# p-m-mueller/saddle_point_petsc

Hardware: AMD Instinct MI355X
Metric: FGMRES iterations/sec + achieved HBM GB/s on A-block SpMV, 1/2/4/8 MI355X (higher is better)
Workload: dtype f64

## Files before the change

### saddle_point_petsc_amd/csrc/spk_dict.hpp

```cpp
#pragma once
#include "spk_device.hpp"

namespace spk {
namespace k {

constexpr int kDictChunk = kThreads;
constexpr int kDictG3 = 9;
constexpr int kDict2Wgs = 512;
typedef int int2v __attribute__((ext_vector_type(2)));
typedef unsigned long long u64;

struct DictArgs {
    const uint16_t *tid;
    const int32_t *tab;
    const double *cls;
    const int32_t *fld;
    const unsigned char *codes;
    const double *zpad;
    int32_t nbrows, ntype, nclass, kmax;
    int32_t nchunks, chunks_per_xcd, chunks_per_wg;
    int32_t tab_ints, cls_off, fld_off;
    int64_t plane_off[kDictMaxK];
    int32_t strad;
    int32_t u3l[9], u3r[9];
    int32_t uw[4];
};

__device__ __forceinline__ void dict_load_lds(const DictArgs &d, int nclsvals, char *smem)
{
    int32_t *ti = reinterpret_cast<int32_t *>(smem);
    for (int i = threadIdx.x; i < d.tab_ints; i += blockDim.x) ti[i] = d.tab[i];
    double2 *cv = reinterpret_cast<double2 *>(smem + d.cls_off);
    const double2 *src = reinterpret_cast<const double2 *>(d.cls);
    for (int i = threadIdx.x; i < nclsvals; i += blockDim.x) cv[i] = src[i];
    int32_t *fl = reinterpret_cast<int32_t *>(smem + d.fld_off);
    for (int i = threadIdx.x; i < nclsvals; i += blockDim.x) fl[i] = d.fld[i];
    __syncthreads();
}
struct DictTables {
    const int32_t *tlen;
    int2 *tent;
    const double2 *cv;
    const int32_t *fl;
};
__device__ __forceinline__ DictTables dict_tables(const DictArgs &d, char *smem)
{
    return DictTables{reinterpret_cast<const int32_t *>(smem), reinterpret_cast<int2 *>(smem + 4 * ((d.ntype + 1) & ~1)),
                      reinterpret_cast<const double2 *>(smem + d.cls_off), reinterpret_cast<const int32_t *>(smem + d.fld_off)};
}
__device__ __forceinline__ bool dict_chunk_range(const DictArgs &d, int bx, int &c0, int &c1)
{
    c0 = ((bx & 7) * d.chunks_per_xcd + (bx >> 3) * d.chunks_per_wg);
    c1 = min(min(c0 + d.chunks_per_wg, ((bx & 7) + 1) * d.chunks_per_xcd), d.nchunks);
    return c0 < c1;
}
template <int KM>
__device__ __forceinline__ void dict_prepare_types(const DictArgs &d, const DictTables &T, int stride)
{
    for (int i = threadIdx.x; i < d.ntype * KM; i += kThreads) {
        const int t = i / KM, k = i - t * KM;
        int2 e = T.tent[i];
        if (k < T.tlen[t]) e.x *= stride;
        else e = make_int2((int)0x80000000u, d.nclass);
        T.tent[i] = e;
    }
    __syncthreads();
}
__device__ __forceinline__ int dict_rowof(const DictArgs &d, int ch) { return min(ch * kDictChunk + (int)threadIdx.x, d.nbrows - 1); }

__device__ __forceinline__ void dict_issue_pair2(const DictArgs &d, int p, int64_t br, u64 &w0, u64 &w1)
{
    const unsigned char *base = d.codes + d.plane_off[p];
    if (2 * p + 1 < d.kmax) {
        const int4v r = __builtin_nontemporal_load(reinterpret_cast<const int4v *>(base) + br);
        w0 = (u64)(uint32_t)r.x | ((u64)(uint32_t)r.y << 32);
        w1 = (u64)(uint32_t)r.z | ((u64)(uint32_t)r.w << 32);
    } else {
        const int2v r = __builtin_nontemporal_load(reinterpret_cast<const int2v *>(base) + br);
        w0 = (u64)(uint32_t)r.x | ((u64)(uint32_t)r.y << 32);
        w1 = 0ull;
    }
}
__device__ __forceinline__ void dict_issue3(const DictArgs &d, int k, int64_t br, u64 &w0, u64 &w1)
{
    const int4v r = __builtin_nontemporal_load(reinterpret_cast<const int4v *>(d.codes + d.plane_off[k]) + br);
    w0 = (u64)(uint32_t)r.x | ((u64)(uint32_t)r.y << 32);
    w1 = (u64)(uint32_t)r.z | ((u64)(uint32_t)r.w << 32);
}
__device__ __forceinline__ int dict_field(u64 w0, u64 w1, int fd)
{
    const u64 w = (fd >> 16) ? w1 : w0;
    const int sh = fd & 255, wd = (fd >> 8) & 255;
    return (int)((long long)(w << (64 - sh - wd)) >> (64 - wd));
}
template <int SPLIT>
__device__ __forceinline__ constexpr bool dict3_in_w1(int e)
{
    return SPLIT == 1 ? e >= 5 : SPLIT == 2 ? e >= 4 : (e == 4 || e >= 6);
}
template <int SPLIT>
__device__ __forceinline__ int dict_field3u(u64 w0, u64 w1, const DictArgs &d, int e)
{
    const u64 w = dict3_in_w1<SPLIT>(e) ? w1 : w0;
    return (int)((long long)(w << d.u3l[e]) >> 32) >> d.u3r[e];
}
__device__ __forceinline__ int dict_field2(u64 w, int fd)
{
    const int lo = (int)(uint32_t)w, hi = (int)(uint32_t)(w >> 32);
    const int mask = fd >> 31;
    const int src = (hi & mask) | (lo & ~mask);
    return __builtin_amdgcn_sbfe(src, (unsigned)fd, (unsigned)(fd >> 8));
}
constexpr int kDictAcross = 1 << 30;
__device__ __forceinline__ int dict_field2(u64 w, int fd, bool strad)
{
    if (strad && (fd & kDictAcross)) {
        const int sh = fd & 63, wd = (fd >> 8) & 31;
        return (int)((long long)(w << (64 - sh - wd)) >> (64 - wd));
    }
    return dict_field2(w, fd);
}
__device__ __forceinline__ double dict_decode(int code, double2 bs)
{
    return __builtin_fma((double)code, bs.y, bs.x);
}
template <int BS>
__device__ __forceinline__ u64 *dict_word_ptr(const DictArgs &d, unsigned char *codes, int k, int64_t br)
{
    if (BS == 3) return reinterpret_cast<u64 *>(codes + d.plane_off[k]) + 2 * br;
    const int p = k >> 1;
    if (2 * p + 1 < d.kmax) return reinterpret_cast<u64 *>(codes + d.plane_off[p]) + 2 * br + (k & 1);
    return reinterpret_cast<u64 *>(codes + d.plane_off[p]) + br;
}

inline DictArgs dict_args(const DictDev &A, int *grid)
{
    DictArgs d{};
    d.tid = A.tid.p;
    d.tab = A.tab.p;
    d.cls = A.cls.p;
    d.fld = A.fld.p;
    d.codes = A.codes.p;
    d.zpad = A.zpad.p;
    d.strad = A.straddle ? 1 : 0;
    for (int e = 0; e < 9; ++e) {
        d.u3l[e] = A.u3l[e];
        d.u3r[e] = A.u3r[e];
    }
    for (int e = 0; e < 4; ++e) d.uw[e] = A.uniform ? A.uw[e] : 0;
    d.nbrows = A.nbrows;
    d.ntype = A.ntype;
    d.nclass = A.nclass;
    d.kmax = A.kmax;
    d.nchunks = (A.nbrows + kDictChunk - 1) / kDictChunk;
    static const int wgs2 = [] { const char *e = getenv("SPK_DICT2_WGS"); return e && atoi(e) > 0 ? atoi(e) : kDict2Wgs; }();
    d.chunks_per_wg = std::max(1, d.nchunks / (A.bs == 2 && A.kmax == 9 ? wgs2 : 2048));
    const int cpx = (d.nchunks + 7) / 8;
    d.chunks_per_xcd = (cpx + d.chunks_per_wg - 1) / d.chunks_per_wg * d.chunks_per_wg;
    d.tab_ints = ((A.ntype + 1) & ~1) + 2 * A.ntype * A.kmax;
    d.cls_off = (4 * d.tab_ints + 15) & ~15;
    d.fld_off = d.cls_off + 16 * (A.nclass + 1) * A.bs * A.bs;
    for (int k = 0; k < kDictMaxK; ++k) d.plane_off[k] = A.plane_off[k];
    *grid = 8 * (d.chunks_per_xcd / d.chunks_per_wg);
    return d;
}

}
}
```

### saddle_point_petsc_amd/csrc/spk_k_dict.hip

```cpp
#include "spk_dict.hpp"

#include <climits>

namespace spk {
namespace k {

template <int BS, bool ACC, bool RIDE, bool BT, int U3>
__global__ __launch_bounds__(kThreads) void spmv_dict_kernel(DictArgs d, const double *__restrict__ x, double *__restrict__ y,
                                                             RowTail tail, const int32_t *__restrict__ done, GivensRider gr)
{
#pragma clang fp contract(off)
    extern __shared__ __attribute__((aligned(16))) char smem[];
    const int bx = product_prologue<RIDE>(done, gr, reinterpret_cast<double *>(smem));
    int c0, c1;
    if (bx < 0 || !dict_chunk_range(d, bx, c0, c1)) return;
    int br = c0 * kDictChunk + (int)threadIdx.x;
    int tidn = br < d.nbrows ? (int)d.tid[br] : -1;
    dict_load_lds(d, (d.nclass + 1) * BS * BS, smem);
    const DictTables T = dict_tables(d, smem);

    for (int ch = c0; ch < c1; ++ch) {
        const int tc = tidn;
        const int brc = br;
        br += kDictChunk;
        tidn = (ch + 1 < c1 && br < d.nbrows) ? (int)d.tid[br] : -1;
        if (tc < 0) continue;
        double s[BS];
#pragma unroll
        for (int r = 0; r < BS; ++r) s[r] = 0.0;
        double yacc[BS];
        if (ACC) {
            if (BS == 2) {
                const double2 t = reinterpret_cast<const double2 *>(y)[brc];
                yacc[0] = t.x;
                yacc[1] = t.y;
            } else {
#pragma unroll
                for (int r = 0; r < BS; ++r) yacc[r] = y[(int64_t)BS * brc + r];
            }
        }
        BtPre pre[BS];
        if (BT) {
#pragma unroll
            for (int r = 0; r < BS; ++r) pre[r].load(tail, (int64_t)BS * brc + r);
        }
        const int len = T.tlen[tc];
        const int2 *te = T.tent + (size_t)tc * d.kmax;
        constexpr int G = BS == 2 ? 10 : kDictG3;
        for (int k0 = 0; k0 < len; k0 += G) {
            int2 e[G];
            u64 w0[G], w1[BS == 2 ? 1 : G];
            double xv[G][BS];
            if (BS == 2) {
#pragma unroll
                for (int h = 0; h < G / 2; ++h) {
                    w0[2 * h] = w0[2 * h + 1] = 0ull;
                    if (k0 + 2 * h < len) dict_issue_pair2(d, (k0 >> 1) + h, brc, w0[2 * h], w0[2 * h + 1]);
                }
            }
#pragma unroll
            for (int g = 0; g < G; ++g) {
                const bool in = k0 + g < len;
                e[g] = in ? te[k0 + g] : make_int2(0, 0);
                if (in) {
                    if (BS == 3) dict_issue3(d, k0 + g, brc, w0[g], w1[BS == 2 ? 0 : g]);
                    const int64_t c = (int64_t)brc + e[g].x;
                    if (BS == 2) {
                        const double2 t = reinterpret_cast<const double2 *>(x)[c];
                        xv[g][0] = t.x;
                        xv[g][1] = t.y;
                    } else {
#pragma unroll
                        for (int j = 0; j < BS; ++j) xv[g][j] = x[BS * c + j];
                    }
                }
            }
#pragma unroll
            for (int g = 0; g < G; ++g) {
                if (k0 + g < len) {
                    const double2 *cb = T.cv + (size_t)e[g].y * (BS * BS);
                    const int32_t *fb = T.fl + (size_t)e[g].y * (BS * BS);
#pragma unroll
                    for (int r = 0; r < BS; ++r)
#pragma unroll
                        for (int j = 0; j < BS; ++j)
                            s[r] += dict_decode(BS == 2 ? dict_field2(w0[g], fb[r * BS + j], d.strad != 0)
                                                       : U3 ? dict_field3u<(U3 ? U3 : 1)>(w0[g], w1[BS == 2 ? 0 : g], d, r * BS + j)
                                                            : dict_field(w0[g], w1[BS == 2 ? 0 : g], fb[r * BS + j]),
                                                cb[r * BS + j]) * xv[g][j];
                }
            }
        }
#pragma unroll
        for (int r = 0; r < BS; ++r) {
            row_tail_add(tail, (int64_t)BS * brc + r, s[r], false);
            if (BT) pre[r].add(tail, s[r]);
            if (ACC) s[r] += yacc[r];
        }
        if (BS == 2) {
            double2 o;
            o.x = s[0];
            o.y = s[1];
            reinterpret_cast<double2 *>(y)[brc] = o;
        } else {
#pragma unroll
            for (int r = 0; r < BS; ++r) y[(int64_t)BS * brc + r] = s[r];
        }
    }
}

template <int KM, bool ACC>
struct Dict2Stage {
    u64 w[KM + 1];
    double2 xv[KM];
    int cls[KM];
    double2 yv;
};

template <int KM, bool ACC>
__device__ __forceinline__ void dict2_issue(const DictArgs &d, __amdgpu_buffer_rsrc_t xr, const double *__restrict__ y,
                                            const int2 *tent, int tc, int brr, Dict2Stage<KM, ACC> &S)
{
    static_assert(KM % 2 == 1, "an odd last position: its plane holds single words");
#pragma unroll
    for (int h = 0; h < KM / 2; ++h) {
        const int4v r = __builtin_nontemporal_load(reinterpret_cast<const int4v *>(d.codes + d.plane_off[h]) + brr);
        S.w[2 * h] = (u64)(uint32_t)r.x | ((u64)(uint32_t)r.y << 32);
        S.w[2 * h + 1] = (u64)(uint32_t)r.z | ((u64)(uint32_t)r.w << 32);
    }
    {
        const int2v r = __builtin_nontemporal_load(reinterpret_cast<const int2v *>(d.codes + d.plane_off[KM / 2]) + brr);
        S.w[KM - 1] = (u64)(uint32_t)r.x | ((u64)(uint32_t)r.y << 32);
    }
    if (ACC) S.yv = reinterpret_cast<const double2 *>(y)[brr];
    const int2 *te = tent + (size_t)tc * KM;
    const uint32_t b16 = (uint32_t)brr * 16u;
#pragma unroll
    for (int g = 0; g < KM; ++g) {
        const int2 e = te[g];
        S.cls[g] = e.y;
        const int4v r = __builtin_bit_cast(int4v, __builtin_amdgcn_raw_buffer_load_b128(xr, (int)(b16 + (uint32_t)e.x), 0, 0));
        S.xv[g].x = __hiloint2double(r.y, r.x);
        S.xv[g].y = __hiloint2double(r.w, r.z);
    }
}

template <bool ACC, bool RIDE, bool BT, int KM, bool UNI>
__global__ __launch_bounds__(kThreads) void spmv_dict2_kernel(DictArgs d, const double *__restrict__ x, double *__restrict__ y,
                                                              RowTail tail, const int32_t *__restrict__ done, GivensRider gr)
{
#pragma clang fp contract(off)
    extern __shared__ __attribute__((aligned(16))) char smem[];
    const int bx = product_prologue<RIDE>(done, gr, reinterpret_cast<double *>(smem));
    int c0, c1;
    if (bx < 0 || !dict_chunk_range(d, bx, c0, c1)) return;
    int tA = (int)d.tid[dict_rowof(d, c0)];
    int tB = (int)d.tid[dict_rowof(d, c0 + 1)];
    dict_load_lds(d, (d.nclass + 1) * 4, smem);
    const DictTables T = dict_tables(d, smem);
    dict_prepare_types<KM>(d, T, 16);
    const __amdgpu_buffer_rsrc_t xr = __builtin_amdgcn_make_buffer_rsrc(const_cast<double *>(x), 0, 16 * d.nbrows, 0x00020000);

    Dict2Stage<KM, ACC> SA, SB;
    auto compute = [&](int ch, const Dict2Stage<KM, ACC> &S) {
        const int brc = ch * kDictChunk + (int)threadIdx.x;
        double s[2] = {0.0, 0.0};
#pragma unroll
        for (int g = 0; g < KM; ++g) {
            const double2 *cb = T.cv + (size_t)S.cls[g] * 4;
            if (UNI) {
                const int lo = (int)(uint32_t)S.w[g], hi = (int)(uint32_t)(S.w[g] >> 32);
                s[0] += dict_decode(__builtin_amdgcn_sbfe(lo, 0u, (unsigned)d.uw[0]), cb[0]) * S.xv[g].x;
                s[0] += dict_decode(lo >> (32 - d.uw[1]), cb[1]) * S.xv[g].y;
                s[1] += dict_decode(__builtin_amdgcn_sbfe(hi, 0u, (unsigned)d.uw[2]), cb[2]) * S.xv[g].x;
                s[1] += dict_decode(hi >> (32 - d.uw[3]), cb[3]) * S.xv[g].y;
            } else {
                const int32_t *fb = T.fl + (size_t)S.cls[g] * 4;
                s[0] += dict_decode(dict_field2(S.w[g], fb[0]), cb[0]) * S.xv[g].x;
                s[0] += dict_decode(dict_field2(S.w[g], fb[1]), cb[1]) * S.xv[g].y;
                s[1] += dict_decode(dict_field2(S.w[g], fb[2]), cb[2]) * S.xv[g].x;
                s[1] += dict_decode(dict_field2(S.w[g], fb[3]), cb[3]) * S.xv[g].y;
            }
        }
        if (brc >= d.nbrows) return;
#pragma unroll
        for (int r = 0; r < 2; ++r) {
            row_tail_add(tail, 2 * (int64_t)brc + r, s[r], BT);
            if (ACC) s[r] += r == 0 ? S.yv.x : S.yv.y;
        }
        double2 o;
        o.x = s[0];
        o.y = s[1];
        reinterpret_cast<double2 *>(y)[brc] = o;
    };

    dict2_issue<KM, ACC>(d, xr, y, T.tent, tA, dict_rowof(d, c0), SA);
    tA = (int)d.tid[dict_rowof(d, c0 + 2)];
    for (int ch = c0;; ch += 2) {
        dict2_issue<KM, ACC>(d, xr, y, T.tent, tB, dict_rowof(d, ch + 1), SB);
        tB = (int)d.tid[dict_rowof(d, ch + 3)];
        compute(ch, SA);
        if (ch + 1 >= c1) break;
        dict2_issue<KM, ACC>(d, xr, y, T.tent, tA, dict_rowof(d, ch + 2), SA);
        tA = (int)d.tid[dict_rowof(d, ch + 4)];
        compute(ch + 1, SB);
        if (ch + 2 >= c1) break;
    }
}

void spmv_dict(const DictDev &A, const double *x, double *y, const CsrDev *bt, const double *lam, const int32_t *done,
               hipStream_t s, bool accumulate, const OffDiag *odp, const GivensRider *rider)
{
    if (product_is_empty(A.nbrows, rider, done, s)) return;
    if (spmv_dict3(A, x, y, bt, lam, done, s, accumulate, odp, rider)) return;
    const ProductLaunch p = make_product_launch(bt, lam, odp, rider, done, accumulate);
    int grid = 0;
    const DictArgs d = dict_args(A, &grid);
    const size_t lds = std::max((size_t)A.lds_bytes, p.rider_lds);
    const bool pipelined = A.bs == 2 && A.kmax == 9 && A.nbrows < (1 << 27) && !A.straddle;
    dispatch_product(p.acc, p.ride, p.bt, [&](auto acc, auto ride, auto btf) {
        constexpr bool ACC = acc.value, RIDE = ride.value, BTF = btf.value;
        auto launch = [&](auto kern) {
            SPK_LAUNCH_PRODUCT(kern, dim3(grid + p.nride), dim3(kThreads), lds, s, d, x, y, p.tail, p.done, p.gr);
        };
        if (pipelined && A.uniform) launch(spmv_dict2_kernel<ACC, RIDE, BTF, 9, true>);
        else if (pipelined) launch(spmv_dict2_kernel<ACC, RIDE, BTF, 9, false>);
        else if (A.bs == 2) launch(spmv_dict_kernel<2, ACC, RIDE, BTF, 0>);
        else if (A.uniform3 == 0) launch(spmv_dict_kernel<3, ACC, RIDE, BTF, 0>);
        else if (A.uniform3 == 1) launch(spmv_dict_kernel<3, ACC, RIDE, BTF, 1>);
        else if (A.uniform3 == 2) launch(spmv_dict_kernel<3, ACC, RIDE, BTF, 2>);
        else launch(spmv_dict_kernel<3, ACC, RIDE, BTF, 3>);
    });
}

template <int BS, int U3>
__global__ __launch_bounds__(kThreads) void jacobi_sweep_f32_dict_kernel(DictArgs d, const float *__restrict__ d32, float omega,
                                                                         const float *__restrict__ x32,
                                                                         const float *__restrict__ yin, float *__restrict__ yout,
                                                                         const int32_t *__restrict__ done)
{
#pragma clang fp contract(off)
    if (done && *done) return;
    extern __shared__ __attribute__((aligned(16))) char smem[];
    int c0, c1;
    if (!dict_chunk_range(d, (int)blockIdx.x, c0, c1)) return;
    dict_load_lds(d, (d.nclass + 1) * BS * BS, smem);
    const DictTables T = dict_tables(d, smem);
    for (int ch = c0; ch < c1; ++ch) {
        const int br = ch * kDictChunk + (int)threadIdx.x;
        if (br >= d.nbrows) continue;
        const int tc = (int)d.tid[br];
        float s[BS];
#pragma unroll
        for (int r = 0; r < BS; ++r) s[r] = 0.0f;
        const int len = T.tlen[tc];
        const int2 *te = T.tent + (size_t)tc * d.kmax;
        constexpr int G = BS == 2 ? 10 : 3;
        for (int k0 = 0; k0 < len; k0 += G) {
            int2 e[G];
            u64 w0[G], w1[BS == 2 ? 1 : G];
            float yv[G][BS];
            if (BS == 2) {
#pragma unroll
                for (int h = 0; h < G / 2; ++h) {
                    w0[2 * h] = w0[2 * h + 1] = 0ull;
                    if (k0 + 2 * h < len) dict_issue_pair2(d, (k0 >> 1) + h, br, w0[2 * h], w0[2 * h + 1]);
                }
            }
#pragma unroll
            for (int g = 0; g < G; ++g) {
                const bool in = k0 + g < len;
                e[g] = in ? te[k0 + g] : make_int2(0, 0);
                if (in) {
                    if (BS == 3) dict_issue3(d, k0 + g, br, w0[g], w1[BS == 2 ? 0 : g]);
                    const int64_t c = (int64_t)br + e[g].x;
#pragma unroll
                    for (int j = 0; j < BS; ++j) yv[g][j] = yin[BS * c + j];
                }
            }
#pragma unroll
            for (int g = 0; g < G; ++g) {
                if (k0 + g < len) {
                    const double2 *cb = T.cv + (size_t)e[g].y * (BS * BS);
                    const int32_t *fb = T.fl + (size_t)e[g].y * (BS * BS);
#pragma unroll
                    for (int r = 0; r < BS; ++r)
#pragma unroll
                        for (int j = 0; j < BS; ++j)
                            s[r] = (s[r] + ((float)dict_decode(BS == 2 ? dict_field2(w0[g], fb[r * BS + j], d.strad != 0)
                                                                      : U3 ? dict_field3u<(U3 ? U3 : 1)>(w0[g], w1[BS == 2 ? 0 : g], d, r * BS + j)
                                                                           : dict_field(w0[g], w1[BS == 2 ? 0 : g], fb[r * BS + j]),
                                                               cb[r * BS + j]) * yv[g][j]));
                }
            }
        }
#pragma unroll
        for (int r = 0; r < BS; ++r) {
            const int64_t row = (int64_t)BS * br + r;
            yout[row] = sweep_update(yin[row], omega, d32[row], x32[row], s[r]);
        }
    }
}

void jacobi_sweep_f32_dict(const DictDev &A, const float *d32, float omega, const float *x32, const float *yin, float *yout,
                           const int32_t *done, hipStream_t s)
{
    if (A.nbrows == 0) return;
    if (jacobi_sweep_f32_dict3(A, d32, omega, x32, yin, yout, done, s)) return;
    int grid = 0;
    const DictArgs d = dict_args(A, &grid);
#define SPK_LAUNCH_SWEEP(BS, U3)                                                                                                \
    hipLaunchKernelGGL((jacobi_sweep_f32_dict_kernel<BS, U3>), dim3(grid), dim3(kThreads), (size_t)A.lds_bytes, s, d, d32, omega, x32, \
                       yin, yout, done)
    if (A.bs == 2) SPK_LAUNCH_SWEEP(2, 0);
    else if (A.uniform3 == 0) SPK_LAUNCH_SWEEP(3, 0);
    else if (A.uniform3 == 1) SPK_LAUNCH_SWEEP(3, 1);
    else if (A.uniform3 == 2) SPK_LAUNCH_SWEEP(3, 2);
    else SPK_LAUNCH_SWEEP(3, 3);
#undef SPK_LAUNCH_SWEEP
}

__device__ __forceinline__ unsigned long long mix64(unsigned long long h, unsigned long long w)
{
    h ^= w + 0x9E3779B97F4A7C15ull + (h << 6) + (h >> 2);
    h *= 0xBF58476D1CE4E5B9ull;
    h ^= h >> 31;
    return h;
}
__device__ __forceinline__ int dict_insert(unsigned long long h, int32_t item, unsigned long long *keys, int32_t *rep,
                                           int32_t *ctl, int maxkeys)
{
    if (h == 0ull) h = 1ull;
    int idx = (int)(h & (unsigned long long)(kDictSlots - 1));
    for (int probe = 0; probe < kDictSlots; ++probe) {
        if (__hip_atomic_load(ctl + 1, __ATOMIC_RELAXED, __HIP_MEMORY_SCOPE_AGENT)) return -1;
        unsigned long long prev = __hip_atomic_load(keys + idx, __ATOMIC_RELAXED, __HIP_MEMORY_SCOPE_AGENT);
        if (prev == 0ull) {
            prev = atomicCAS(keys + idx, 0ull, h);
            if (prev == 0ull && atomicAdd(ctl, 1) + 1 > maxkeys) {
                __hip_atomic_store(ctl + 1, 1, __ATOMIC_RELAXED, __HIP_MEMORY_SCOPE_AGENT);
                return -1;
            }
        }
        if (prev == 0ull || prev == h) {
            if (item < __hip_atomic_load(rep + idx, __ATOMIC_RELAXED, __HIP_MEMORY_SCOPE_AGENT)) atomicMin(rep + idx, item);
            return idx;
        }
        idx = (idx + 1) & (kDictSlots - 1);
    }
    __hip_atomic_store(ctl + 1, 1, __ATOMIC_RELAXED, __HIP_MEMORY_SCOPE_AGENT);
    return -1;
}

template <int BS>
__device__ __forceinline__ double blk_val(const double *v0, const double *v1, int64_t ldp, int64_t q, int r, int j)
{
    if (BS == 2) return (r == 0 ? v0 : v1)[2 * q + j];
    return v0[(int64_t)(3 * r + j) * ldp + q];
}
__device__ __forceinline__ unsigned long long coarse_key(double v)
{
    if (!(fabs(v) < 1e12)) return (unsigned long long)__double_as_longlong(v);
    return (unsigned long long)(long long)rint(v * 1048576.0);
}

template <int BS>
__global__ __launch_bounds__(kThreads) void dict_hash_blocks_kernel(const double *__restrict__ v0, const double *__restrict__ v1,
                                                                    int64_t ldp, int64_t nblocks, unsigned long long *keys,
                                                                    int32_t *rep, int32_t *slot, int32_t *ctl, int maxkeys)
{
    const int64_t q = (int64_t)blockIdx.x * kThreads + threadIdx.x;
    if (q >= nblocks) return;
    unsigned long long h = 0x243F6A8885A308D3ull;
#pragma unroll
    for (int r = 0; r < BS; ++r)
#pragma unroll
        for (int j = 0; j < BS; ++j) h = mix64(h, coarse_key(blk_val<BS>(v0, v1, ldp, q, r, j)));
    slot[q] = dict_insert(h, (int32_t)q, keys, rep, ctl, maxkeys);
}
void dict_hash_blocks(int bs, const double *v0, const double *v1, int64_t ldp, int64_t nblocks, unsigned long long *keys,
                      int32_t *rep, int32_t *slot, int32_t *ctl, int maxkeys, hipStream_t s)
{
    if (nblocks == 0) return;
    const unsigned grid = (unsigned)((nblocks + kThreads - 1) / kThreads);
    if (bs == 2) hipLaunchKernelGGL((dict_hash_blocks_kernel<2>), dim3(grid), dim3(kThreads), 0, s, v0, v1, ldp, nblocks, keys, rep, slot, ctl, maxkeys);
    else hipLaunchKernelGGL((dict_hash_blocks_kernel<3>), dim3(grid), dim3(kThreads), 0, s, v0, v1, ldp, nblocks, keys, rep, slot, ctl, maxkeys);
}

template <int BS>
__global__ __launch_bounds__(kThreads) void dict_cls_base_kernel(const double *__restrict__ v0, const double *__restrict__ v1,
                                                                 int64_t ldp, const int32_t *__restrict__ rep_of_id, int nid,
                                                                 double *__restrict__ cls)
{
    const int i = blockIdx.x * kThreads + threadIdx.x;
    if (i >= nid * BS * BS) return;
    const int id = i / (BS * BS), e = i % (BS * BS);
    cls[2 * i] = blk_val<BS>(v0, v1, ldp, rep_of_id[id], e / BS, e % BS);
    cls[2 * i + 1] = 1.0;
}
template <int BS>
__global__ __launch_bounds__(kThreads) void dict_cls_stats_kernel(const double *__restrict__ v0, const double *__restrict__ v1,
                                                                  int64_t ldp, int64_t nblocks, const int32_t *__restrict__ slot2id,
                                                                  int32_t *__restrict__ slot, const double *__restrict__ cls,
                                                                  int32_t *__restrict__ gexp, unsigned long long *__restrict__ dmax,
                                                                  int32_t *__restrict__ bad)
{
    const int64_t q = (int64_t)blockIdx.x * kThreads + threadIdx.x;
    if (q >= nblocks) return;
    const int sl = slot[q];
    const int id = sl >= 0 ? slot2id[sl] : -1;
    slot[q] = id;
    if (id < 0) {
        *bad = 1;
        return;
    }
#pragma unroll
    for (int r = 0; r < BS; ++r)
#pragma unroll
        for (int j = 0; j < BS; ++j) {
            const int e = r * BS + j;
            const double v = blk_val<BS>(v0, v1, ldp, q, r, j), base = cls[2 * (id * BS * BS + e)];
            const double dv = v - base;
            if (__double_as_longlong(base + dv) != __double_as_longlong(v) || !(fabs(dv) < 1e300)) {
                *bad = 1;
                continue;
            }
            if (dv == 0.0) continue;
            const unsigned long long bits = (unsigned long long)__double_as_longlong(fabs(dv));
            const int ef = (int)(bits >> 52);
            const unsigned long long mant = (bits & 0xFFFFFFFFFFFFFull) | (ef ? 0x10000000000000ull : 0ull);
            const int low = (ef ? ef - 1075 : -1074) + (int)__builtin_ctzll(mant);
            if (low < __hip_atomic_load(gexp + id * BS * BS + e, __ATOMIC_RELAXED, __HIP_MEMORY_SCOPE_AGENT)) atomicMin(gexp + id * BS * BS + e, low);
            if (bits > __hip_atomic_load(dmax + id * BS * BS + e, __ATOMIC_RELAXED, __HIP_MEMORY_SCOPE_AGENT)) atomicMax(dmax + id * BS * BS + e, bits);
        }
}
void dict_class_stats(int bs, const double *v0, const double *v1, int64_t ldp, int64_t nblocks, const int32_t *rep_of_id, int nid,
                      const int32_t *slot2id, int32_t *slot, double *cls, int32_t *gexp, unsigned long long *dmax, int32_t *bad,
                      hipStream_t s)
{
    if (nblocks == 0 || nid == 0) return;
    const unsigned g1 = (unsigned)((nid * bs * bs + kThreads - 1) / kThreads), g2 = (unsigned)((nblocks + kThreads - 1) / kThreads);
    if (bs == 2) {
        hipLaunchKernelGGL((dict_cls_base_kernel<2>), dim3(g1), dim3(kThreads), 0, s, v0, v1, ldp, rep_of_id, nid, cls);
        hipLaunchKernelGGL((dict_cls_stats_kernel<2>), dim3(g2), dim3(kThreads), 0, s, v0, v1, ldp, nblocks, slot2id, slot, cls, gexp, dmax, bad);
    } else {
        hipLaunchKernelGGL((dict_cls_base_kernel<3>), dim3(g1), dim3(kThreads), 0, s, v0, v1, ldp, rep_of_id, nid, cls);
        hipLaunchKernelGGL((dict_cls_stats_kernel<3>), dim3(g2), dim3(kThreads), 0, s, v0, v1, ldp, nblocks, slot2id, slot, cls, gexp, dmax, bad);
    }
}

__global__ __launch_bounds__(kThreads) void dict_hash_rows_kernel(const int32_t *__restrict__ browptr, const int32_t *__restrict__ bcol,
                                                                  const int32_t *__restrict__ blkid, int32_t nbrows,
                                                                  unsigned long long *keys, int32_t *rep, int32_t *slot, int32_t *ctl,
                                                                  int maxkeys, int kmax)
{
    const int br = blockIdx.x * kThreads + threadIdx.x;
    if (br >= nbrows) return;
    const int q0 = browptr[br], q1 = browptr[br + 1];
    if (q1 - q0 > kmax) {
        __hip_atomic_store(ctl + 1, 1, __ATOMIC_RELAXED, __HIP_MEMORY_SCOPE_AGENT);
        slot[br] = -1;
        return;
    }
    unsigned long long h = mix64(0x13198A2E03707344ull, (unsigned long long)(q1 - q0));
    for (int q = q0; q < q1; ++q)
        h = mix64(h, ((unsigned long long)(uint32_t)(bcol[q] - br) << 32) | (unsigned long long)(uint32_t)blkid[q]);
    slot[br] = dict_insert(h, br, keys, rep, ctl, maxkeys);
}
void dict_hash_rows(const int32_t *browptr, const int32_t *bcol, const int32_t *blkid, int32_t nbrows, unsigned long long *keys,
                    int32_t *rep, int32_t *slot, int32_t *ctl, int maxkeys, int kmax, hipStream_t s)
{
    if (nbrows == 0) return;
    hipLaunchKernelGGL(dict_hash_rows_kernel, dim3((nbrows + kThreads - 1) / kThreads), dim3(kThreads), 0, s, browptr, bcol, blkid,
                       nbrows, keys, rep, slot, ctl, maxkeys, kmax);
}

__global__ __launch_bounds__(kThreads) void dict_row_table_kernel(const int32_t *__restrict__ browptr, const int32_t *__restrict__ bcol,
                                                                  const int32_t *__restrict__ blkid, const int32_t *__restrict__ rep_of_id,
                                                                  int nid, int kmax, int32_t *__restrict__ tab)
{
    const int i = blockIdx.x * kThreads + threadIdx.x;
    if (i >= nid * kmax) return;
    const int id = i / kmax, k = i % kmax;
    const int br = rep_of_id[id];
    const int q0 = browptr[br], len = browptr[br + 1] - q0;
    if (k == 0) tab[id] = len;
    int32_t *ent = tab + ((nid + 1) & ~1) + 2 * (size_t)i;
    ent[0] = k < len ? bcol[q0 + k] - br : 0;
    ent[1] = k < len ? blkid[q0 + k] : 0;
}
__global__ __launch_bounds__(kThreads) void dict_row_verify_kernel(const int32_t *__restrict__ browptr, const int32_t *__restrict__ bcol,
                                                                   const int32_t *__restrict__ blkid, int32_t nbrows, int nid, int kmax,
                                                                   const int32_t *__restrict__ slot2id, const int32_t *__restrict__ slot,
                                                                   const int32_t *__restrict__ tab, uint16_t *__restrict__ tid,
                                                                   int32_t *__restrict__ bad)
{
    const int br = blockIdx.x * kThreads + threadIdx.x;
    if (br >= nbrows) return;
    const int sl = slot[br];
    const int id = sl >= 0 ? slot2id[sl] : -1;
    bool same = id >= 0;
    if (same) {
        const int q0 = browptr[br], len = browptr[br + 1] - q0;
        same = len == tab[id];
        const int32_t *ent = tab + ((nid + 1) & ~1) + 2 * (size_t)id * kmax;
        for (int k = 0; same && k < len; ++k) same = ent[2 * k] == bcol[q0 + k] - br && ent[2 * k + 1] == blkid[q0 + k];
    }
    if (!same) *bad = 1;
    tid[br] = (uint16_t)(same ? id : 0);
}
void dict_fill_rows(const int32_t *browptr, const int32_t *bcol, const int32_t *blkid, int32_t nbrows, const int32_t *rep_of_id,
                    int nid, int kmax, const int32_t *slot2id, const int32_t *slot, int32_t *tab, uint16_t *tid, int32_t *bad,
                    hipStream_t s)
{
    if (nbrows == 0 || nid == 0) return;
    hipLaunchKernelGGL(dict_row_table_kernel, dim3((nid * kmax + kThreads - 1) / kThreads), dim3(kThreads), 0, s, browptr, bcol, blkid,
                       rep_of_id, nid, kmax, tab);
    hipLaunchKernelGGL(dict_row_verify_kernel, dim3((nbrows + kThreads - 1) / kThreads), dim3(kThreads), 0, s, browptr, bcol, blkid,
                       nbrows, nid, kmax, slot2id, slot, tab, tid, bad);
}

template <int BS>
__global__ __launch_bounds__(kThreads) void dict_encode_kernel(DictArgs d, const int32_t *__restrict__ browptr,
                                                               const int32_t *__restrict__ blkid, const double *__restrict__ v0,
                                                               const double *__restrict__ v1, int64_t ldp, unsigned char *__restrict__ codes,
                                                               int32_t *__restrict__ bad)
{
    const int64_t br = (int64_t)blockIdx.x * kThreads + threadIdx.x;
    if (br >= d.nbrows) return;
    const int q0 = browptr[br], len = browptr[br + 1] - q0;
    for (int k = 0; k < len; ++k) {
        const int id = blkid[q0 + k];
        u64 w[2] = {0ull, 0ull};
#pragma unroll
        for (int r = 0; r < BS; ++r)
#pragma unroll
            for (int j = 0; j < BS; ++j) {
                const int e = r * BS + j;
                const double base = d.cls[2 * (id * BS * BS + e)], sc = d.cls[2 * (id * BS * BS + e) + 1];
                const int fd = d.fld[id * BS * BS + e];
                const int wd = BS == 2 ? (fd >> 8) & 31 : (fd >> 8) & 255;
                const int sh = BS == 2 ? ((fd & kDictAcross) ? (fd & 63) : (fd & 31) + ((fd >> 31) & 1) * 32) : (fd & 255);
                const int wi = BS == 2 ? 0 : (fd >> 16);
                const double kq = (blk_val<BS>(v0, v1, ldp, q0 + k, r, j) - base) / sc;
                const long long kk = (long long)rint(kq);
                const long long lim = 1ll << (wd - 1);
                if ((double)kk != kq || kk < -lim || kk > lim - 1) *bad = 1;
                w[wi] |= ((u64)kk & ((wd >= 64) ? ~0ull : ((1ull << wd) - 1ull))) << sh;
            }
        u64 *p = dict_word_ptr<BS>(d, codes, k, br);
        p[0] = w[0];
        if (BS == 3) p[1] = w[1];
    }
}
template <int BS>
__global__ __launch_bounds__(kThreads) void dict_verify_kernel(DictArgs d, const int32_t *__restrict__ browptr,
                                                               const int32_t *__restrict__ bcol, const double *__restrict__ v0,
                                                               const double *__restrict__ v1, int64_t ldp, int32_t *__restrict__ bad)
{
    const int64_t br = (int64_t)blockIdx.x * kThreads + threadIdx.x;
    if (br >= d.nbrows) return;
    const int t = d.tid[br];
    const int q0 = browptr[br], len = browptr[br + 1] - q0;
    const int32_t *ent = d.tab + ((d.ntype + 1) & ~1) + 2 * (size_t)t * d.kmax;
    bool ok = t < d.ntype && d.tab[t] == len;
    for (int k = 0; ok && k < len; ++k) {
        u64 w0 = 0ull, w1 = 0ull;
        if (BS == 2) {
            u64 a0, a1;
            dict_issue_pair2(d, k >> 1, br, a0, a1);
            w0 = (k & 1) ? a1 : a0;
        } else {
            dict_issue3(d, k, br, w0, w1);
        }
        ok = ok && bcol[q0 + k] == (int)br + ent[2 * k];
        const int cls_id = ent[2 * k + 1];
        const double2 *cb = reinterpret_cast<const double2 *>(d.cls) + (size_t)cls_id * (BS * BS);
        const int32_t *fb = d.fld + (size_t)cls_id * (BS * BS);
#pragma unroll
        for (int r = 0; r < BS; ++r)
#pragma unroll
            for (int j = 0; j < BS; ++j)
                ok = ok && __double_as_longlong(dict_decode(BS == 2 ? dict_field2(w0, fb[r * BS + j], d.strad != 0) : dict_field(w0, w1, fb[r * BS + j]), cb[r * BS + j])) ==
                               __double_as_longlong(blk_val<BS>(v0, v1, ldp, q0 + k, r, j));
    }
    if (!ok) *bad = 1;
}
void dict_encode_verify(const DictDev &A, const int32_t *browptr, const int32_t *bcol, const int32_t *blkid, const double *v0,
                        const double *v1, int64_t ldp, int32_t *bad, hipStream_t s)
{
    if (A.nbrows == 0) return;
    int grid = 0;
    const DictArgs d = dict_args(A, &grid);
    const unsigned g = (unsigned)((A.nbrows + kThreads - 1) / kThreads);
    if (A.bs == 2) {
        hipLaunchKernelGGL((dict_encode_kernel<2>), dim3(g), dim3(kThreads), 0, s, d, browptr, blkid, v0, v1, ldp, A.codes.p, bad);
        hipLaunchKernelGGL((dict_verify_kernel<2>), dim3(g), dim3(kThreads), 0, s, d, browptr, bcol, v0, v1, ldp, bad);
    } else {
        hipLaunchKernelGGL((dict_encode_kernel<3>), dim3(g), dim3(kThreads), 0, s, d, browptr, blkid, v0, v1, ldp, A.codes.p, bad);
        hipLaunchKernelGGL((dict_verify_kernel<3>), dim3(g), dim3(kThreads), 0, s, d, browptr, bcol, v0, v1, ldp, bad);
    }
}

}
}
```

Before: 6845.

## Overlap dict2 table setup with first code stream loads and use buffer ops for y

The pipelined bs=2 dictionary SpMV kernel now issues the first chunk's code-plane and y loads before the LDS tables are built. When the tables fit in one value per thread, it loads them directly into registers and commits them with a single barrier instead of two strided LDS passes. Global y loads and stores become raw buffer loads and stores, so out-of-range rows are dropped by the buffer bounds check rather than by a branch. The row-tail add is skipped when no tail exists, and row indices are clamped to the workgroup's own chunk range. This shortens the kernel prologue, but it depends on buffer bounds handling for correctness on padded rows.

```diff
diff --git a/saddle_point_petsc_amd/csrc/spk_dict.hpp b/saddle_point_petsc_amd/csrc/spk_dict.hpp
--- a/saddle_point_petsc_amd/csrc/spk_dict.hpp
+++ b/saddle_point_petsc_amd/csrc/spk_dict.hpp
@@ -67,6 +67,36 @@
     __syncthreads();
 }
 __device__ __forceinline__ int dict_rowof(const DictArgs &d, int ch) { return min(ch * kDictChunk + (int)threadIdx.x, d.nbrows - 1); }
+__device__ __forceinline__ int dict_rowof(const DictArgs &d, int ch, int c1)
+{
+    return min(ch < c1 ? ch * kDictChunk + (int)threadIdx.x : c1 * kDictChunk - 1, d.nbrows - 1);
+}
+
+template <int KM, bool UNI>
+struct Dict2TableWords {
+    int2 ent;
+    int len, fl;
+    double2 cv;
+    __device__ __forceinline__ static bool fits(const DictArgs &d) { return d.ntype * KM <= kThreads && (d.nclass + 1) * 4 <= kThreads; }
+    __device__ __forceinline__ void request(const DictArgs &d)
+    {
+        const int e = min((int)threadIdx.x, d.ntype * KM - 1), c = min((int)threadIdx.x, (d.nclass + 1) * 4 - 1);
+        ent = reinterpret_cast<const int2 *>(d.tab + ((d.ntype + 1) & ~1))[e];
+        len = d.tab[e / KM];
+        cv = reinterpret_cast<const double2 *>(d.cls)[c];
+        fl = UNI ? 0 : d.fld[c];
+    }
+    __device__ __forceinline__ void commit(const DictArgs &d, const DictTables &T, int stride) const
+    {
+        const int i = threadIdx.x;
+        if (i < d.ntype * KM) T.tent[i] = i % KM < len ? make_int2(ent.x * stride, ent.y) : make_int2((int)0x80000000u, d.nclass);
+        if (i < (d.nclass + 1) * 4) {
+            const_cast<double2 *>(T.cv)[i] = cv;
+            if (!UNI) const_cast<int32_t *>(T.fl)[i] = fl;
+        }
+        __syncthreads();
+    }
+};
 
 __device__ __forceinline__ void dict_issue_pair2(const DictArgs &d, int p, int64_t br, u64 &w0, u64 &w1)
 {
diff --git a/saddle_point_petsc_amd/csrc/spk_k_dict.hip b/saddle_point_petsc_amd/csrc/spk_k_dict.hip
--- a/saddle_point_petsc_amd/csrc/spk_k_dict.hip
+++ b/saddle_point_petsc_amd/csrc/spk_k_dict.hip
@@ -116,10 +116,10 @@
     int cls[KM];
     double2 yv;
 };
+typedef decltype(__builtin_amdgcn_raw_buffer_load_b128(__amdgpu_buffer_rsrc_t(), 0, 0, 0)) b128_t;
 
 template <int KM, bool ACC>
-__device__ __forceinline__ void dict2_issue(const DictArgs &d, __amdgpu_buffer_rsrc_t xr, const double *__restrict__ y,
-                                            const int2 *tent, int tc, int brr, Dict2Stage<KM, ACC> &S)
+__device__ __forceinline__ void dict2_issue_stream(const DictArgs &d, __amdgpu_buffer_rsrc_t yr, int brr, Dict2Stage<KM, ACC> &S)
 {
     static_assert(KM % 2 == 1, "an odd last position: its plane holds single words");
 #pragma unroll
@@ -132,7 +132,15 @@
         const int2v r = __builtin_nontemporal_load(reinterpret_cast<const int2v *>(d.codes + d.plane_off[KM / 2]) + brr);
         S.w[KM - 1] = (u64)(uint32_t)r.x | ((u64)(uint32_t)r.y << 32);
     }
-    if (ACC) S.yv = reinterpret_cast<const double2 *>(y)[brr];
+    if (ACC) {
+        const int4v r = __builtin_bit_cast(int4v, __builtin_amdgcn_raw_buffer_load_b128(yr, (int)((uint32_t)brr * 16u), 0, 0));
+        S.yv.x = __hiloint2double(r.y, r.x);
+        S.yv.y = __hiloint2double(r.w, r.z);
+    }
+}
+template <int KM, bool ACC>
+__device__ __forceinline__ void dict2_issue_gather(__amdgpu_buffer_rsrc_t xr, const int2 *tent, int tc, int brr, Dict2Stage<KM, ACC> &S)
+{
     const int2 *te = tent + (size_t)tc * KM;
     const uint32_t b16 = (uint32_t)brr * 16u;
 #pragma unroll
@@ -154,14 +162,26 @@
     const int bx = product_prologue<RIDE>(done, gr, reinterpret_cast<double *>(smem));
     int c0, c1;
     if (bx < 0 || !dict_chunk_range(d, bx, c0, c1)) return;
-    int tA = (int)d.tid[dict_rowof(d, c0)];
-    int tB = (int)d.tid[dict_rowof(d, c0 + 1)];
-    dict_load_lds(d, (d.nclass + 1) * 4, smem);
+    const bool has_tail = BT || tail.od.rowptr != nullptr;
+    int tA = (int)d.tid[dict_rowof(d, c0, c1)];
+    int tB = (int)d.tid[dict_rowof(d, c0 + 1, c1)];
     const DictTables T = dict_tables(d, smem);
-    dict_prepare_types<KM>(d, T, 16);
     const __amdgpu_buffer_rsrc_t xr = __builtin_amdgcn_make_buffer_rsrc(const_cast<double *>(x), 0, 16 * d.nbrows, 0x00020000);
-
+    const __amdgpu_buffer_rsrc_t yr = __builtin_amdgcn_make_buffer_rsrc(y, 0, 16 * d.nbrows, 0x00020000);
+    Dict2TableWords<KM, UNI> tw;
+    tw.request(d);
+    __builtin_amdgcn_sched_barrier(0);
     Dict2Stage<KM, ACC> SA, SB;
+    dict2_issue_stream<KM, ACC>(d, yr, dict_rowof(d, c0, c1), SA);
+    if (Dict2TableWords<KM, UNI>::fits(d)) {
+        tw.commit(d, T, 16);
+    } else {
+        dict_load_lds(d, (d.nclass + 1) * 4, smem);
+        dict_prepare_types<KM>(d, T, 16);
+    }
+    dict2_issue_gather<KM, ACC>(xr, T.tent, tA, dict_rowof(d, c0, c1), SA);
+    tA = (int)d.tid[dict_rowof(d, c0 + 2, c1)];
+
     auto compute = [&](int ch, const Dict2Stage<KM, ACC> &S) {
         const int brc = ch * kDictChunk + (int)threadIdx.x;
         double s[2] = {0.0, 0.0};
@@ -182,27 +202,30 @@
                 s[1] += dict_decode(dict_field2(S.w[g], fb[3]), cb[3]) * S.xv[g].y;
             }
         }
-        if (brc >= d.nbrows) return;
-#pragma unroll
-        for (int r = 0; r < 2; ++r) {
-            row_tail_add(tail, 2 * (int64_t)brc + r, s[r], BT);
-            if (ACC) s[r] += r == 0 ? S.yv.x : S.yv.y;
+        if (has_tail && brc < d.nbrows) {
+#pragma unroll
+            for (int r = 0; r < 2; ++r) row_tail_add(tail, 2 * (int64_t)brc + r, s[r], BT);
+        }
+        if (ACC) {
+            s[0] += S.yv.x;
+            s[1] += S.yv.y;
         }
         double2 o;
         o.x = s[0];
         o.y = s[1];
-        reinterpret_cast<double2 *>(y)[brc] = o;
+        __builtin_amdgcn_raw_buffer_store_b128(__builtin_bit_cast(b128_t, o), yr, (int)((uint32_t)brc * 16u), 0, 0);
     };
-
-    dict2_issue<KM, ACC>(d, xr, y, T.tent, tA, dict_rowof(d, c0), SA);
-    tA = (int)d.tid[dict_rowof(d, c0 + 2)];
+    auto issue = [&](int ch, int &t, Dict2Stage<KM, ACC> &S) {
+        dict2_issue_stream<KM, ACC>(d, yr, dict_rowof(d, ch, c1), S);
+        dict2_issue_gather<KM, ACC>(xr, T.tent, t, dict_rowof(d, ch, c1), S);
+        t = (int)d.tid[dict_rowof(d, ch + 2, c1)];
+        __builtin_amdgcn_sched_barrier(0);
+    };
     for (int ch = c0;; ch += 2) {
-        dict2_issue<KM, ACC>(d, xr, y, T.tent, tB, dict_rowof(d, ch + 1), SB);
-        tB = (int)d.tid[dict_rowof(d, ch + 3)];
+        issue(ch + 1, tB, SB);
         compute(ch, SA);
         if (ch + 1 >= c1) break;
-        dict2_issue<KM, ACC>(d, xr, y, T.tent, tA, dict_rowof(d, ch + 2), SA);
-        tA = (int)d.tid[dict_rowof(d, ch + 4)];
+        issue(ch + 2, tA, SA);
         compute(ch + 1, SB);
         if (ch + 2 >= c1) break;
     }
```

New measurement: 7008 (median of 6 runs). 1.02x the previous value.
